# DiltheyLab/HLA-LA

Measured on AMD Instinct MI355X. Metric: paired reads/sec aligned to PRG graph, higher is better.
Workload: dtype int32

## Files before the change

hla-la_amd/csrc/kernel_dp.hip:

```cpp
#include "batch.h"
#include "../../include/hlala_gpu.h"

namespace hlala {

enum { K_DIAG = 0, K_GGAP = 1, K_SGAP = 2, K_HOP = 3, K_JUMP = 4 };
enum { M_D = 0, M_GG = 1, M_SG = 2 };
enum { PH_IDLE = 0, PH_RUN, PH_SELECT, PH_BT, PH_EXPAND, PH_DONE };

constexpr u64 HKEY_EMPTY = ~0ull;
#ifndef HLALA_DP_PROFILE_LOG2
#define HLALA_DP_PROFILE_LOG2 18
#endif
#ifndef HLALA_EARLY_GEN_MAX
#define HLALA_EARLY_GEN_MAX 0xFFFFFE
#endif
constexpr int DP_EARLY_GEN_MAX = HLALA_EARLY_GEN_MAX;
constexpr int EXT_PENDING = 0x7FFFFFFF;
constexpr int DP_BT_STEPS_PER_TRIP = 32;

#ifndef HLALA_DP_TAIL_THREADS
#define HLALA_DP_TAIL_THREADS 128
#endif
constexpr int DP_TAIL_THREADS = HLALA_DP_TAIL_THREADS;
#ifndef HLALA_DP_TINY_WAVES
#define HLALA_DP_TINY_WAVES 4
#endif
#ifndef HLALA_DP_WIDE_THREADS
#define HLALA_DP_WIDE_THREADS 64
#endif
#ifndef HLALA_DP_BROAD_THREADS
#define HLALA_DP_BROAD_THREADS HLALA_DP_TAIL_THREADS
#endif
#ifndef HLALA_DP_LARGE_THREADS
#define HLALA_DP_LARGE_THREADS HLALA_DP_TAIL_THREADS
#endif
#ifndef HLALA_DP_HUGE_THREADS
#define HLALA_DP_HUGE_THREADS HLALA_DP_TAIL_THREADS
#endif
struct DpTiny  { static constexpr bool JF = false; static constexpr int THREADS = 64, WAVES = HLALA_DP_TINY_WAVES, GW = 16, WCAP = 16,   HC = 32,   IBITS = 4,  CELLS = 2048,     EARLY = 4096,     IMPCAP = 64,   COMPLETED = 256,          STEPS = 1024;     typedef u32 Best; typedef short Slot; typedef unsigned char ImpIdx; static constexpr bool IN_MEMORY = false; };
#ifndef HLALA_DP_TINYJF_WAVES
#define HLALA_DP_TINYJF_WAVES 4
#endif
struct DpTinyJF : DpTiny { static constexpr bool JF = true; static constexpr int WAVES = HLALA_DP_TINYJF_WAVES; };
struct DpMid   { static constexpr bool JF = false; static constexpr int THREADS = 64, WAVES = 4, GW = 32, WCAP = 32,   HC = 128,  IBITS = 5,  CELLS = 4096,     EARLY = 8192,     IMPCAP = 256,  COMPLETED = 512,          STEPS = 2048;     typedef u32 Best; typedef short Slot; typedef unsigned short ImpIdx; static constexpr bool IN_MEMORY = false; };
struct DpSmall { static constexpr bool JF = false; static constexpr int THREADS = 64, WAVES = 5, GW = 64, WCAP = 64,   HC = 128,  IBITS = 7,  CELLS = DP_CELLS, EARLY = DP_CELLS, IMPCAP = 2048, COMPLETED = DP_COMPLETED, STEPS = DP_STEPS; typedef u32 Best; typedef short Slot; typedef unsigned short ImpIdx; static constexpr bool IN_MEMORY = false; };
struct DpWide  { static constexpr bool JF = false; static constexpr int THREADS = HLALA_DP_WIDE_THREADS, WAVES = 2, GW = HLALA_DP_WIDE_THREADS, WCAP = 256,  HC = 512,  IBITS = 8,  CELLS = DP_CELLS, EARLY = DP_CELLS, IMPCAP = 2048, COMPLETED = DP_COMPLETED, STEPS = DP_STEPS; typedef u32 Best; typedef short Slot; typedef unsigned short ImpIdx; static constexpr bool IN_MEMORY = false; };
struct DpBroad { static constexpr bool JF = false; static constexpr int THREADS = HLALA_DP_BROAD_THREADS, WAVES = 1, GW = HLALA_DP_BROAD_THREADS, WCAP = 512,  HC = 1024, IBITS = 9,  CELLS = DP_CELLS_LARGE, EARLY = DP_CELLS_LARGE, IMPCAP = 4096, COMPLETED = DP_COMPLETED_LARGE, STEPS = DP_STEPS; typedef u32 Best; typedef int Slot; typedef unsigned short ImpIdx; static constexpr bool IN_MEMORY = false; };
struct DpLarge { static constexpr bool JF = false; static constexpr int THREADS = HLALA_DP_LARGE_THREADS, WAVES = 1, GW = HLALA_DP_LARGE_THREADS, WCAP = 1024, HC = 2048, IBITS = 10, CELLS = DP_CELLS_LARGE, EARLY = DP_CELLS_LARGE, IMPCAP = 4096, COMPLETED = DP_COMPLETED_LARGE, STEPS = DP_STEPS; typedef u32 Best; typedef int Slot; typedef unsigned short ImpIdx; static constexpr bool IN_MEMORY = false; };

struct DpHuge  { static constexpr bool JF = false; static constexpr int THREADS = HLALA_DP_HUGE_THREADS, WAVES = 1, GW = HLALA_DP_HUGE_THREADS, WCAP = 8192, HC = 16384, IBITS = 13, CELLS = 131072, EARLY = 131072, IMPCAP = 8192, COMPLETED = 65536, STEPS = DP_STEPS; typedef u64 Best; typedef int Slot; typedef unsigned short ImpIdx; static constexpr bool IN_MEMORY = true; };
#ifndef HLALA_DP_SORT_SCRATCH
#define HLALA_DP_SORT_SCRATCH 4096
#endif
constexpr int DP_SORT_SCRATCH = HLALA_DP_SORT_SCRATCH;

struct DpState {
    int itemIdx;
    int item, rOff, seqLen, start_seq, startLevel, startNode;
    int d, b1, b2, n1, n2, nCells, nCompleted, curMax, firstMaxSlot, lastInc, earlyInit, itersRun, diagonals;
    int earlyMaxNat;
    u32 cellsEvaluated;
    int endSlot, endScore, nSteps, nCols;
    int have, sb, se, err;
    int isAlias;
    int needTier;
};

template <bool SMALL> struct TlistT { typedef unsigned short type; };
template <> struct TlistT<true> { typedef unsigned char type; };

template <class C>
struct __align__(16) DpLdsT {
    u64 hkey[C::HC];
    typename C::Best hbest[3][C::HC];
    typename TlistT<(C::HC <= 256)>::type tlist[C::HC];
    u64 fkey[2][C::WCAP];
    typename C::Slot fslot[2][C::WCAP];
    short fD[2][C::WCAP], fG[2][C::WCAP], fS[2][C::WCAP];
    typename C::Slot tes[C::HC];
    unsigned char timp[C::HC];
    typename C::ImpIdx hq[C::HC];
    int nNew, nImp, nKeepF, err, nCompletedAdd;
    int chunkNext, chunkEnd;
    int jumpMet;
    int nTa;
    int nextPhase;
    int btSlot, btM, btX, btY, btGuard, btDone;
    DpState st;
    u64 accCalls, accIters, accCells, accEdges;
#ifdef HLALA_DP_TIMING
    long long tPh[16];
#endif
#ifdef HLALA_DP_PROFILE
    long long pfStart; int pfSlow, pfImp, pfPre, pfMaxNT, pfMaxF; long long pfPh[16];
#endif
};

struct __align__(16) CellRec { u64 key; short sc[4]; u32 bt[3]; u32 pad; };

template <class C>
struct DpSlabT {
    char* base;
    static constexpr size_t O_CELL      = 0;
    static constexpr size_t O_EARLY_KEY = O_CELL + (size_t)C::CELLS * 32;
    static constexpr size_t O_STEP_XY   = O_EARLY_KEY + (size_t)C::EARLY * 8;
    static constexpr size_t O_IMP_KEY   = O_STEP_XY + (size_t)C::STEPS * 8;
    static constexpr size_t O_IMP_NEW   = O_IMP_KEY + (size_t)C::IMPCAP * 8;
// ... 127 lines not shown
template <int GW> __device__ __forceinline__ u64 grp_ballot(bool p)
{
    static_assert(GW <= 64, "grp_ballot: one wavefront at most (grp_any / grp_rank for blocks)");
    u64 b = __ballot(p);
    if(GW == 64) return b;
    return (b >> grp_base<GW>()) & ((1ull << (GW & 63)) - 1ull);
}
template <int GW> __device__ __forceinline__ bool grp_any(bool p)
{
    if constexpr (GW > 64) {
        const int w = __ballot(p) != 0 ? 1 : 0; int* x = blk_words<GW>();
        if(lane_id() == 0) x[threadIdx.x >> 6] = w;
        blk_barrier();
        int r = 0;
#pragma unroll
        for(int i = 0; i < BlkX<GW>::NW; i++) r |= x[i];
        blk_barrier();
        return r != 0;
    } else return grp_ballot<GW>(p) != 0;
}
template <int GW> __device__ __forceinline__ int grp_rank(bool p, int& total)
{
    if constexpr (GW > 64) {
        const u64 m = __ballot(p);
        const int off = (int)__builtin_amdgcn_mbcnt_hi((u32)(m >> 32), __builtin_amdgcn_mbcnt_lo((u32)m, 0u));
        int* x = blk_words<GW>(); const int wv = (int)(threadIdx.x >> 6);
        if(lane_id() == 0) x[wv] = __popcll(m);
        blk_barrier();
        int before = 0, tot = 0;
#pragma unroll
        for(int i = 0; i < BlkX<GW>::NW; i++) { const int t = x[i]; if(i < wv) before += t; tot += t; }
        blk_barrier();
        total = tot;
        return before + off;
    } else {
        const u64 m = grp_ballot<GW>(p);
        total = __popcll(m);
        return __popcll(m & ((1ull << grp_lane<GW>()) - 1ull));
    }
}
template <int GW> __device__ __forceinline__ int grp_bcast0(int v)
{
    if(GW == 64) return __builtin_amdgcn_readfirstlane(v);
    if constexpr (GW > 64) {
        int* x = blk_words<GW>();
        if(threadIdx.x == 0) x[0] = v;
        blk_barrier();
        const int r = x[0];
        blk_barrier();
        return __builtin_amdgcn_readfirstlane(r);
    } else return __shfl(v, grp_base<GW>());
}
template <int GW> __device__ __forceinline__ int guni(int v) { return GW >= 64 ? __builtin_amdgcn_readfirstlane(v) : v; }

template <class C> __device__ __forceinline__ void dp_sync()
{
#if defined(__AMDGCN_TGSPLIT__) || defined(__gfx950_tgsplit__)
#error "kernel_dp.hip: dp_sync releases at workgroup scope -- build with -DHLALA_DP_AGENT_RELEASE for threadgroup-split mode"
#endif
#ifdef HLALA_DP_AGENT_RELEASE
#define DP_RELEASE_SCOPE "agent"
#else
#define DP_RELEASE_SCOPE "workgroup"
#endif
    if constexpr (C::IN_MEMORY) { __builtin_amdgcn_fence(__ATOMIC_RELEASE, DP_RELEASE_SCOPE); if constexpr (C::GW > 64) __builtin_amdgcn_s_barrier(); else __builtin_amdgcn_wave_barrier(); __builtin_amdgcn_fence(__ATOMIC_ACQUIRE, "agent"); }
    else if constexpr (C::GW > 64) blk_barrier();
    else { WSYNC(); }
}
#define DSYNC() dp_sync<C>()

__device__ __forceinline__ u64 mk_key(int x, int y, int node) { return ((u64)(u32)x << 40) | ((u64)(u32)y << 28) | (u64)(u32)node; }
__device__ __forceinline__ int key_x(u64 k) { return (int)(k >> 40); }
__device__ __forceinline__ int key_y(u64 k) { return (int)((k >> 28) & 0xFFF); }
__device__ __forceinline__ int key_node(u64 k) { return (int)(k & 0xFFFFFFF); }
__device__ __forceinline__ u32 hash64(u64 k)
{
    const u32 node = (u32)k & 0xFFFFFFFu, y = (u32)(k >> 28) & 0xFFFu, x = (u32)(k >> 40);
    u32 h = node + __umul24(y, 17u) + __umul24(x, 31u);
    return h ^ (h >> 6) ^ (h >> 12);
}

__device__ __forceinline__ u32 hash_mix(u64 k)
{
    u32 h = (u32)k * 0x9E3779B1u ^ (u32)(k >> 32) * 0x85EBCA77u;
    h ^= h >> 15; h *= 0x2C1B3C6Du; h ^= h >> 12;
    return h;
}

template <class C> __device__ __forceinline__ u32 tgt_hash(u64 k) { return (C::HC > 256 ? hash_mix(k) : hash64(k)) & (u32)(C::HC - 1); }

template <class C>
__device__ inline int dp_find(const DpLdsT<C>& S, u64 key)
{
    u32 h = tgt_hash<C>(key);
#pragma nounroll
    for(int probe = 0; probe < C::HC; probe++) {
        const u64 cur = S.hkey[h];
        if(cur == key) return (int)h;
        if(cur == HKEY_EMPTY) return -1;
        h = (h + 1) & (C::HC - 1);
    }
    return -1;
}

__device__ __forceinline__ u32 mk_bt(int prev, int src, int kind, int edge) { return (u32)prev | ((u32)src << 17) | ((u32)kind << 19) | (((u32)edge & 0xFFu) << 22); }
__device__ __forceinline__ int bt_prev(u32 b) { return (int)(b & 0x1FFFF); }
// ... 158 lines not shown
    const int gl = grp_lane<GW>();
    for(int i = gl; i < C::HC; i += GW) { S.hkey[i] = HKEY_EMPTY; S.hbest[0][i] = 0; S.hbest[1][i] = 0; S.hbest[2][i] = 0; }
    if(gl == 0) {
        DpState& st = S.st;
        st.itemIdx = itemIdx;
        st.item = it.item; st.rOff = it.rOff; st.seqLen = it.seqLen; st.start_seq = it.start_seq; st.startLevel = it.startLevel; st.startNode = it.startNode;
        st.diagonals = it.seqLen + G.L - 1;
        st.d = 1; st.b1 = 0; st.b2 = 1; st.n1 = 1; st.n2 = 0; st.nCells = 1; st.nCompleted = 0;
        st.curMax = 0; st.firstMaxSlot = 0; st.lastInc = 0; st.earlyInit = 0; st.earlyMaxNat = -1; st.itersRun = 0;
        st.cellsEvaluated = 0;
        st.endSlot = -1; st.endScore = 0; st.nSteps = 0; st.nCols = 0;
        st.have = 0; st.sb = 0; st.se = -1; st.err = 0; st.needTier = 0; st.isAlias = 0;
        S.err = 0; S.nTa = 0; S.jumpMet = 0;
#ifdef HLALA_DP_PROFILE
        S.pfStart = clock64(); S.pfSlow = 0; S.pfImp = 0; S.pfPre = 0; S.pfMaxNT = 0; S.pfMaxF = 0; for(int i = 0; i < 16; i++) S.pfPh[i] = 0;
#endif
        CellRec c0; c0.key = mk_key(it.startLevel, it.start_seq, it.startNode);
        c0.sc[0] = 0; c0.sc[1] = (short)DP_NEG; c0.sc[2] = (short)DP_NEG; c0.sc[3] = 0; c0.bt[0] = 0; c0.bt[1] = 0; c0.bt[2] = 0; c0.pad = 0;
        sl.cell()[0] = c0;
        S.fkey[0][0] = mk_key(it.startLevel, it.start_seq, it.startNode); S.fslot[0][0] = 0;
        S.fD[0][0] = 0; S.fG[0][0] = (short)DP_NEG; S.fS[0][0] = (short)DP_NEG;
    }
    DSYNC();
    return PH_RUN;
}

template <class C>
__device__ inline int dp_iterate(DpLdsT<C>& S, const DpSlabT<C>& sl, const DevGraph& G, const int4* nrec, const uint8_t* readBases, const bool fwd, int& edgesAcc, u64* sortScratch)
{
    constexpr int GW = C::GW;
    const int gl = grp_lane<GW>();
    DpState& st = S.st;
    const int dir = fwd ? 1 : -1;
    const int seqLen = guni<GW>(st.seqLen);
    const int max_levelI = G.L - 1, max_seqI = seqLen;
    const int limitY = fwd ? seqLen : 0;
    const int d = guni<GW>(st.d);
    const int n1 = guni<GW>(st.n1), n2 = guni<GW>(st.n2);
    const int b1 = guni<GW>(st.b1), b2 = guni<GW>(st.b2), bn = b2;
    const int lastInc0 = guni<GW>(st.lastInc), diagonals = guni<GW>(st.diagonals);
    const uint8_t* seqp = readBases + guni<GW>(st.rOff);

    if(d > diagonals || (d - lastInc0) > 40) return PH_SELECT;
    if(n1 == 0 && n2 == 0) {
        int last = lastInc0 + 40; if(last > diagonals) last = diagonals;
        if(gl == 0) st.itersRun = last;
        DSYNC();
        return PH_SELECT;
    }
    if(d > 60000) { if(gl == 0) { st.itersRun = d; st.err = __LINE__; } DSYNC(); return PH_DONE; }

#if defined(HLALA_DP_TIMING)
    long long tq0 = clock64();
#define DP_TQ(i) do { __builtin_amdgcn_s_waitcnt(0); long long t_ = clock64(); if(gl == 0) S.tPh[i] += t_ - tq0; tq0 = t_; } while(0)
#elif defined(HLALA_DP_PROFILE)
    long long tq0 = clock64();
#define DP_TQ(i) do { __builtin_amdgcn_s_waitcnt(0); long long t_ = clock64(); if(gl == 0) S.pfPh[i] += t_ - tq0; tq0 = t_; } while(0)
#else
#define DP_TQ(i) do { } while(0)
#endif
    const int* eoff = fwd ? G.out_off : G.in_off; const int* eto = fwd ? G.out_to : G.in_from; const uint8_t* elab = fwd ? G.out_label : G.in_label;
    const int* joff = fwd ? G.jf_off : G.jb_off; const int* jnode = fwd ? G.jf_node : G.jb_node; const int* jlvl = fwd ? G.jf_lvl : G.jb_lvl;
    const uint8_t* eprk = fwd ? G.out_prank : G.in_prank; const uint8_t* jprk = fwd ? G.jf_prank : G.jb_prank;
    int edges = 0;
    const int nMax = n1 > n2 ? n1 : n2;
    constexpr bool APPEND = (GW >= 64) && (C::WCAP > 64);
    typedef typename TlistT<(C::HC <= 256)>::type TlT;
    int nTa = 0;
    auto append = [&](const bool claimed, const u32 h) {
        if constexpr (APPEND && GW == 64) {
            const u64 m = __ballot(claimed);
            if(claimed) S.tlist[nTa + (int)__builtin_amdgcn_mbcnt_hi((u32)(m >> 32), __builtin_amdgcn_mbcnt_lo((u32)m, 0u))] = (TlT)h;
            nTa += __popcll(m);
        } else if constexpr (APPEND) {
            const u64 m = __ballot(claimed);
            if(m) {
                int base = 0;
                if(lane_id() == 0) base = atomicAdd(&S.nTa, (int)__popcll(m));
                base = __builtin_amdgcn_readfirstlane(base);
                const int pos = base + (int)__builtin_amdgcn_mbcnt_hi((u32)(m >> 32), __builtin_amdgcn_mbcnt_lo((u32)m, 0u));
                if(claimed && pos < C::HC) S.tlist[pos] = (TlT)h;
            }
        }
    };
    for(int i = gl; i < nMax; i += GW) {
        const bool hasA = i < n2, hasB = i < n1;
        u64 pkA = hasA ? S.fkey[b2][i] : 0, pkB = hasB ? S.fkey[b1][i] : 0;
        const int pxA = key_x(pkA), pyA = key_y(pkA), nodeA = key_node(pkA);
        const int pxB = key_x(pkB), pyB = key_y(pkB), nodeB = key_node(pkB);
        const int nxA = pxA + dir, nyA = pyA + dir;
        const bool doA = hasA && !(nxA > max_levelI || nyA > max_seqI || nxA < 0 || nyA < 0);
        const int pDA = hasA ? (int)S.fD[b2][i] : 0;
        const int pD = hasB ? (int)S.fD[b1][i] : 0, pG = hasB ? (int)S.fG[b1][i] : 0, pS = hasB ? (int)S.fS[b1][i] : 0;
        int4 ra0 = make_int4(0, 0, 0, 0), ra1 = ra0, rb0 = ra0, rb1 = ra0; unsigned char rc = 0;
        if(doA) { ra0 = nrec[2 * (size_t)nodeA]; ra1 = nrec[2 * (size_t)nodeA + 1]; rc = fwd ? seqp[pyA] : seqp[pyA - 1]; }
        if(hasB) { rb0 = nrec[2 * (size_t)nodeB]; rb1 = nrec[2 * (size_t)nodeB + 1]; }
        const int a0 = ra0.x, degA = ra0.y & 0xFFFF, tnA0 = ra0.z, tnA1 = ra0.w;
        const unsigned char labA0 = (unsigned char)(ra1.w & 0xFF), labA1 = (unsigned char)((ra1.w >> 8) & 0xFF);
        const int rkA1 = (ra1.w >> 16) & 1, rkB1 = (rb1.w >> 16) & 1;
        const int e0 = rb0.x, degB = rb0.y & 0xFFFF, tnB0 = rb0.z, tnB1 = rb0.w;
        const int j0 = rb1.x, j1 = j0 + (int)((u32)rb0.y >> 16), jn0 = rb1.y, jx0 = rb1.z;
        const unsigned char labB0 = (unsigned char)(rb1.w & 0xFF), labB1 = (unsigned char)((rb1.w >> 8) & 0xFF);
        DP_TQ(4);
        const int ord0 = (1 << (C::IBITS + 8)) | (i << 8);
        const int nyG = pyB + dir, nxB = pxB + dir;
        const bool okA = doA, okB = hasB;
// ... 316 lines not shown
            if(keep && Dv == curMax0 && diff != 0) anyEqDiff = true;
            if(keep) { if(Dv > itMaxNew) { itMaxNew = Dv; itMaxKey = key; } else if(Dv == itMaxNew && key < itMaxKey) itMaxKey = key; }
            if(act) {
                S.hbest[0][h] = keep ? (typename C::Best)(u32)slot : (typename C::Best)0xFFFFFFFFu;
                S.hbest[1][h] = (typename C::Best)(((u32)(unsigned short)(short)mD) | ((u32)(unsigned short)(short)mG << 16));
                S.hbest[2][h] = (typename C::Best)(u32)(unsigned short)(short)mS;
            }
            DP_TQ(13);
        }
        DSYNC();
    }
    anyEqDiff = grp_any<GW>(anyEqDiff); anyOw = grp_any<GW>(anyOw);
    {
        const int mine = itMaxNew;
        itMaxNew = grp_max_i32<GW>(mine);
        if(itMaxNew > curMax0) itMaxKey = grp_min_u64<GW>(mine == itMaxNew ? itMaxKey : ~0ull);
    }
    DP_TQ(6);
    if(guni<GW>(S.err)) { if(gl == 0) { st.itersRun = d; st.err = __LINE__; } DSYNC(); return PH_DONE; }
    const int nCompletedNew = nCompleted0 + guni<GW>(S.nCompletedAdd);
    if constexpr (!C::JF) {
        int nImp = guni<GW>(S.nImp);
        for(int q = gl; q < nImp; q += GW) {
            int es = sl.imp_slot()[q]; int msk = sl.imp_mask()[q];
            for(int m = 0; m < 3; m++) if(msk & (1 << m)) { sl.cell()[es].sc[m] = sl.imp_new()[4 * q + m]; sl.cell()[es].bt[m] = sl.imp_bt()[3 * q + m]; }
        }
        if(nImp) {
            DSYNC();
            for(int i = gl; i < n1; i += GW) {
                const int ph = dp_find<C>(S, S.fkey[b1][i]);
                if(ph >= 0) { const int q = (int)S.hq[ph]; if(q < C::IMPCAP && q < nImp) { S.fD[b1][i] = sl.imp_new()[4 * q + 0]; S.fG[b1][i] = sl.imp_new()[4 * q + 1]; S.fS[b1][i] = sl.imp_new()[4 * q + 2]; } }
            }
        }
    }
    int curMax = curMax0, lastInc = lastInc0, firstMaxSlot = -1;
    if(itMaxNew > curMax0) {
        curMax = itMaxNew; lastInc = d;
        int fs = -1;
        for(int t = gl; t < nT; t += GW) { int h = S.tlist[t]; if(S.hkey[h] == itMaxKey) fs = (int)S.hbest[0][h]; }
        firstMaxSlot = grp_max_i32<GW>(fs);
    }
    if(anyEqDiff || anyOw) lastInc = d;
    int earlyMaxNat = earlyMaxNat0;
    if constexpr (!C::JF) if(earlyInit) { const int m = grp_max_i32<GW>(earlyNatMax); if(m > earlyMaxNat) earlyMaxNat = m; }

    DP_TQ(1);
    int mx = itMaxNew;
    if constexpr (!C::JF) if(slow) {
        mx = DP_NEG;
        for(int t = gl; t < nT; t += GW) { int h = S.tlist[t]; if((u32)S.hbest[0][h] != 0xFFFFFFFFu) { int v = (short)((u32)S.hbest[1][h] & 0xFFFF); mx = max(mx, v); } }
        mx = grp_max_i32<GW>(mx);
    }
    int nNew = 0;
    for(int t0 = 0; t0 < nT; t0 += GW) {
        int t = t0 + gl;
        bool pass = false; u64 key = 0; int h = 0;
        if(t < nT) { h = S.tlist[t]; key = S.hkey[h]; if((u32)S.hbest[0][h] != 0xFFFFFFFFu) { int v = (short)((u32)S.hbest[1][h] & 0xFFFF); pass = (mx - v) <= 15; } }
        int passTot; const int pos = nNew + grp_rank<GW>(pass, passTot);
        if(pass && pos < C::WCAP) {
            S.fkey[bn][pos] = key; S.fslot[bn][pos] = (typename C::Slot)(int)S.hbest[0][h];
            S.fD[bn][pos] = (short)((u32)S.hbest[1][h] & 0xFFFF); S.fG[bn][pos] = (short)((u32)S.hbest[1][h] >> 16); S.fS[bn][pos] = (short)((u32)S.hbest[2][h] & 0xFFFF);
        }
        nNew += passTot;
    }
    if(nNew > C::WCAP) { if(gl == 0) { st.itersRun = d; st.err = __LINE__; st.needTier = tier_for_frontier(nNew); } DSYNC(); return PH_DONE; }
    DSYNC();
    const bool wideSort = C::WCAP > GW && nNew > GW;
    if(wideSort) for(int t = gl; t < nT; t += GW) { int h = S.tlist[t]; S.hkey[h] = HKEY_EMPTY; S.hbest[0][h] = 0; S.hbest[1][h] = 0; S.hbest[2][h] = 0; }
    if(nNew > 1 && nNew <= GW) {
        const bool act = gl < nNew;
        u64 key = 0; typename C::Slot vs = 0; short vD = 0, vG = 0, vS = 0; int rank = 0;
        if(act) {
            key = S.fkey[bn][gl]; vs = S.fslot[bn][gl]; vD = S.fD[bn][gl]; vG = S.fG[bn][gl]; vS = S.fS[bn][gl];
            for(int u = 0; u < nNew; u++) rank += (S.fkey[bn][u] < key) ? 1 : 0;
        }
        DSYNC();
        if(act) { S.fkey[bn][rank] = key; S.fslot[bn][rank] = vs; S.fD[bn][rank] = vD; S.fG[bn][rank] = vG; S.fS[bn][rank] = vS; }
    } else if(wideSort) {
        DSYNC();
        int Pn = GW * 2; while(Pn < nNew) Pn <<= 1;
        u64* keys; u64* pay;
        if constexpr (C::IN_MEMORY) {
            if(Pn <= DP_SORT_SCRATCH) { keys = sortScratch; pay = sortScratch + DP_SORT_SCRATCH; }
            else { keys = sl.sort_spill(); pay = keys + C::WCAP; }
        } else { keys = &S.fkey[bn][0]; pay = (u64*)&S.hbest[2][0]; }
        auto enc = [](int v) -> u64 { return v == DP_NEG ? 0ull : (u64)(u32)(v + 64); };
        auto dec = [](u64 e) -> short { return e == 0 ? (short)DP_NEG : (short)((int)e - 64); };
        for(int i = gl; i < Pn; i += GW) {
            if(i < nNew) {
                pay[i] = ((u64)(u32)(int)S.fslot[bn][i] << 36) | (enc(S.fD[bn][i]) << 24) | (enc(S.fG[bn][i]) << 12) | enc(S.fS[bn][i]);
                if constexpr (C::IN_MEMORY) keys[i] = S.fkey[bn][i];
            } else { keys[i] = ~0ull; pay[i] = 0; }
        }
        DSYNC();
        for(int k = 2; k <= Pn; k <<= 1)
            for(int j = k >> 1; j > 0; j >>= 1) {
                for(int idx = gl; idx < (Pn >> 1); idx += GW) {
                    const int i = ((idx & ~(j - 1)) << 1) | (idx & (j - 1)), l = i | j;
                    const bool up = (i & k) == 0;
                    const u64 ka = keys[i], kb = keys[l];
                    if((ka > kb) == up) { const u64 pa = pay[i], pb = pay[l]; keys[i] = kb; keys[l] = ka; pay[i] = pb; pay[l] = pa; }
                }
                if constexpr (C::IN_MEMORY) { if(Pn <= DP_SORT_SCRATCH) { if constexpr (GW > 64) blk_barrier(); else { WSYNC(); } } else DSYNC(); }
                else DSYNC();
            }
        for(int i = gl; i < Pn; i += GW) {
            const u64 pv = pay[i];
            if(i < nNew) {
                S.fD[bn][i] = dec((pv >> 24) & 0xFFF); S.fG[bn][i] = dec((pv >> 12) & 0xFFF); S.fS[bn][i] = dec(pv & 0xFFF); S.fslot[bn][i] = (typename C::Slot)(int)(pv >> 36);
                if constexpr (C::IN_MEMORY) S.fkey[bn][i] = keys[i];
            }
            if constexpr (!C::IN_MEMORY) pay[i] = 0;
        }
    }
    DSYNC();
    if(!wideSort) for(int t = gl; t < nT; t += GW) { int h = S.tlist[t]; S.hkey[h] = HKEY_EMPTY; S.hbest[0][h] = 0; S.hbest[1][h] = 0; S.hbest[2][h] = 0; }
    if(gl == 0) {
        st.b2 = b1; st.b1 = bn;
        st.n2 = n1; st.n1 = nNew;
        st.d = d + 1; st.itersRun = d;
        st.nCells = nCells; st.nCompleted = nCompletedNew; st.earlyInit = earlyInit; st.earlyMaxNat = earlyMaxNat;
        st.curMax = curMax; st.lastInc = lastInc; if(firstMaxSlot >= 0) st.firstMaxSlot = firstMaxSlot;
        st.cellsEvaluated += (u32)nT;
#ifdef HLALA_DP_PROFILE
        if(slow) S.pfSlow++; S.pfImp += S.nImp; if(prepass) S.pfPre++; if(nT > S.pfMaxNT) S.pfMaxNT = nT; if(nNew > S.pfMaxF) S.pfMaxF = nNew;
#endif
    }
    DSYNC();
    DP_TQ(2);
    return PH_RUN;
}

template <class C>
__device__ inline int dp_select_many(const DpSlabT<C>& sl, const DevGraph& G, int nCompleted, int best, int selectedIndex)
{
    constexpr int GW = C::GW;
    const int gl = grp_lane<GW>();
    int found = -1;
    int nt = 0;
    for(int i0 = 0; i0 < nCompleted; i0 += GW) {
        int i = i0 + gl; bool tie = false; int s = 0; u64 kk = 0;
        if(i < nCompleted) { s = sl.completed()[i]; if(sl.cell()[s].sc[0] == best) { tie = true; u64 k = sl.cell()[s].key; kk = xz_key(key_x(k), key_node(k) - G.level_off[key_x(k)]); } }
        int tieTot; const int rk = grp_rank<GW>(tie, tieTot);
        if(tie) { const int pos = nt + rk; sl.tie_slot()[pos] = s; sl.tie_key()[pos] = kk; }
        nt += tieTot;
    }
    dp_sync<C>();
    u64 prefix = 0; int k = selectedIndex;
    for(int bit = 51; bit >= 0; bit--) {
        int cnt = 0;
        for(int i = gl; i < nt; i += GW) { const u64 kk = sl.tie_key()[i]; if((kk >> (bit + 1)) == (prefix >> (bit + 1)) && !((kk >> bit) & 1ull)) cnt++; }
        cnt = grp_sum_i32<GW>(cnt);
        if(k >= cnt) { k -= cnt; prefix |= 1ull << bit; }
    }
    for(int i = gl; i < nt; i += GW) if(sl.tie_key()[i] == prefix) found = sl.tie_slot()[i];
    return found;
}

template <class C>
__device__ inline int dp_select(DpLdsT<C>& S, const DpSlabT<C>& sl, const DevGraph& G, u32 rng_seed, const bool fwd)
{
    constexpr int GW = C::GW;
    const int gl = grp_lane<GW>();
    DpState& st = S.st;
    const int nCompleted = guni<GW>(st.nCompleted);
    const u32 seed = rng_seed + (u32)guni<GW>(st.item);
    const int curMax = guni<GW>(st.curMax), firstMaxSlot = guni<GW>(st.firstMaxSlot), start_seq = guni<GW>(st.start_seq);
    int endSlot = -1, endScore = 0;
    if(GW <= 64 && nCompleted > 0 && nCompleted <= GW) {
// ... 324 lines not shown
    const DpItem* items[DP_POOL_MAX];
    const uint8_t* bases[DP_POOL_MAX];
};

template <class C, int TIER>
__device__ __forceinline__ void dp_class_run(const DevGraph& G, const DevBatch& B, const DpItem* __restrict__ items, DpLdsT<C>& S, DpSlabT<C> sl, u64* sortScratch, const u32 rng_seed,
                                             const int4* __restrict__ nrecOut, const int4* __restrict__ nrecIn, const uint8_t* __restrict__ readBases);

template <class C, int TIER>
__global__ __launch_bounds__(C::THREADS, C::WAVES) void k_dp(const DevGraph* __restrict__ Gp, const DevBatch* __restrict__ Bp, const DpItem* __restrict__ items,
                                                        char* slabs, size_t slabBytes, u32 rng_seed,
                                                        const int4* __restrict__ nrecOut, const int4* __restrict__ nrecIn, const uint8_t* __restrict__ readBasesArg, const DpPoolArgs pool)
{
    constexpr int GW = C::GW;
    constexpr int NG = GW >= 64 ? 1 : 64 / GW;
    static_assert(C::THREADS == (GW >= 64 ? GW : 64), "block size");
    const DevGraph& G = *Gp;
    const int g = (int)((threadIdx.x & 63) / GW);
    DpLdsT<C>* Sp; DpSlabT<C> sl; u64* sortScratch = nullptr;
    if constexpr (C::IN_MEMORY) {
        __shared__ u64 scratch[2 * DP_SORT_SCRATCH];
        char* base = slabs + (size_t)blockIdx.x * slabBytes;
        Sp = (DpLdsT<C>*)base; sl.base = base + ((sizeof(DpLdsT<C>) + 255) & ~(size_t)255); sortScratch = scratch;
    } else {
        __shared__ DpLdsT<C> SS[NG];
        Sp = &SS[g]; sl.base = slabs + ((size_t)blockIdx.x * NG + g) * slabBytes;
    }
    if constexpr (TIER >= DP_POOL_TIER) {
        const int nB = __builtin_amdgcn_readfirstlane(pool.n);
        for(int bi = 0; bi < nB; bi++) {
            dp_class_run<C, TIER>(G, *pool.B[bi], pool.items[bi], *Sp, sl, sortScratch, pool.seed[bi], nrecOut, nrecIn, pool.bases[bi]);
            DSYNC();
        }
    } else dp_class_run<C, TIER>(G, *Bp, items, *Sp, sl, sortScratch, rng_seed, nrecOut, nrecIn, readBasesArg);
}

template <class C, int TIER>
__device__ __forceinline__ void dp_class_run(const DevGraph& G, const DevBatch& B, const DpItem* __restrict__ items, DpLdsT<C>& S, DpSlabT<C> sl, u64* sortScratch, const u32 rng_seed,
                                             const int4* __restrict__ nrecOut, const int4* __restrict__ nrecIn, const uint8_t* __restrict__ readBases)
{
    constexpr int GW = C::GW;
    constexpr int NG = GW >= 64 ? 1 : 64 / GW;
#ifndef HLALA_DP_DRAW0
#define HLALA_DP_DRAW0 8
#endif
    constexpr int DRAW = (TIER == 0 && C::JF) ? HLALA_DP_DRAW0 : 1;
    const int gl = grp_lane<GW>();

    if(gl == 0) { S.accCalls = 0; S.accIters = 0; S.accCells = 0; S.accEdges = 0; }
#ifdef HLALA_DP_TIMING
    if(gl == 0) { for(int i = 0; i < 16; i++) S.tPh[i] = 0; }
#endif
#ifdef HLALA_DP_TIMING
    long long tAcc[6] = {0, 0, 0, 0, 0, 0}; long long trips = 0, runGroups = 0; long long tMark = clock64();
#define DP_T(i) do { long long t_ = clock64(); tAcc[i] += t_ - tMark; tMark = t_; } while(0)
#else
#define DP_T(i) do { } while(0)
#endif

    constexpr int NPASS = (TIER == 0 && !C::JF) ? 4 : 2;
    for(int pass = 0; pass < NPASS; pass++) {
        const int dirPass = pass & 1;
        const bool foPass = pass >= 2;
        int* fetchCounter = foPass ? &B.work_counter[WC_FO_FETCH + dirPass]
                          : &B.work_counter[TIER == 0 ? (C::JF ? 4 + dirPass : (dirPass ? 10 : 1)) : 13 + 4 * (TIER - 1) + 2 * dirPass];
        const int seg = (C::JF ? DPL_JF : DPL_GEN) + dirPass;
        const bool dense = TIER == 0 && !foPass;
        const int segStart = dense ? uni(B.dp_blk[(size_t)seg * B.dp_nblk]) : 0;
        const int nItems = dense ? uni(B.dp_blk[(size_t)(seg + 1) * B.dp_nblk]) - segStart
                         : (foPass ? uni(B.work_counter[WC_FO_COUNT + dirPass]) : uni(B.work_counter[12 + 4 * (TIER > 0 ? TIER - 1 : 0) + 2 * dirPass]));
        const int* srcList = dense ? B.dp_list + segStart
                           : (foPass ? B.retry_list + (size_t)(14 + dirPass) * (size_t)B.n_chains
                           : B.retry_list + (size_t)(2 * (TIER > 0 ? TIER - 1 : 0) + dirPass) * (size_t)B.n_chains);
        const bool fwd = dirPass != 0;
        if constexpr (DRAW > 1) { if(gl == 0) { S.chunkNext = 0; S.chunkEnd = 0; } DSYNC(); }
        int phase = PH_IDLE;
        bool more = true;
        int edgesAcc = 0;

        for(;;) {
            if(phase == PH_RUN) phase = dp_iterate<C>(S, sl, G, fwd ? nrecOut : nrecIn, readBases, fwd, edgesAcc, sortScratch);
            DP_T(5);
            if(phase == PH_SELECT) phase = dp_select<C>(S, sl, G, rng_seed, fwd);
            DP_T(4);
            if(phase == PH_BT) phase = dp_backtrace<C>(S, sl, DP_BT_STEPS_PER_TRIP, fwd);
            DP_T(3);
            if(phase == PH_EXPAND) phase = dp_expand<C>(S, sl, G, B, fwd ? nrecOut : nrecIn, fwd);
            DP_T(2);
            if(phase == PH_DONE) {
                const int edges = grp_sum_i32<GW>(edgesAcc);
                if(gl == 0) {
                    DpState& st = S.st;
                    S.nextPhase = PH_IDLE;
#ifdef HLALA_DP_PROFILE
                    if(B.dbg && TIER == HLALA_DP_PROFILE && !C::JF) {
                        const long long cyc = clock64() - S.pfStart;
                        if(cyc > (1ll << HLALA_DP_PROFILE_LOG2) && (HLALA_DP_PROFILE_LOG2 >= 12 || (((u32)st.item * 2654435761u) >> 24) == 0)) { int q = atomicAdd(&B.dbg[0], 1); if(q < 500) { int* r = B.dbg + 16 + 16 * q; r[0] = st.item; r[1] = st.itersRun; r[2] = (int)st.cellsEvaluated; r[3] = st.nCells;
                            r[4] = S.pfSlow; r[5] = S.pfImp; r[6] = S.pfPre; r[7] = (int)(cyc >> 10); r[8] = S.pfMaxNT;
                            r[9] = (int)(S.pfPh[4] >> 10); r[10] = (int)(S.pfPh[5] >> 10); r[11] = (int)(S.pfPh[0] >> 10); r[12] = (int)(S.pfPh[3] >> 10); r[13] = (int)(S.pfPh[6] >> 10); r[14] = (int)(S.pfPh[1] >> 10); r[15] = (int)(S.pfPh[2] >> 10); } }
                    }
#endif
                    const bool capacity = st.err != 0 && st.err > -1000000;
                    bool handed = false;
                    if constexpr (C::JF && TIER == 0) if(capacity && S.jumpMet) {
                        if(st.isAlias) ((int*)(items + st.itemIdx))[0] = st.item;
                        const int q = atomicAdd(&B.work_counter[WC_FO_COUNT + dirPass], 1); B.retry_list[(size_t)(14 + dirPass) * (size_t)B.n_chains + q] = st.itemIdx;
                        atomicAdd(&B.work_counter[WC_JF_FAILED], 1);
                        handed = true;
                    }
                    if(handed) { }
                    else if(capacity && TIER < DP_LAST_TIER) {
                        int to = TIER + 1; if(st.needTier > to) to = st.needTier; if(to > DP_LAST_TIER) to = DP_LAST_TIER;
                        int* cnt = &B.work_counter[12 + 4 * (to - 1) + 2 * dirPass]; int* lst = B.retry_list + (size_t)(2 * (to - 1) + dirPass) * (size_t)B.n_chains;
                        if(st.isAlias) ((int*)(items + st.itemIdx))[0] = st.item;
                        int q = atomicAdd(cnt, 1); lst[q] = st.itemIdx;
                        if(to >= DP_SIDE_TIER && B.n_pairs > 0 && !B.unpaired) B.pair_deferred[B.chain_read[st.item >> 1] >> 1] = 1;
                    } else {
                        const int item = st.item;
                        B.dp_iters[item] = st.itersRun; B.dp_score[item] = st.have ? st.endScore : INT32_MIN;
                        B.dp_ncols[item] = st.have ? st.nCols : -1; B.dp_sb[item] = st.sb; B.dp_se[item] = st.se; B.dp_err[item] = st.err;
                        S.accCalls++; S.accIters += (u64)st.itersRun; S.accCells += (u64)st.cellsEvaluated; S.accEdges += (u64)edges;
                        int nx = B.dp_alias_head[item]; if(nx < 0) nx = B.dp_alias_next[item];
                        const bool failed = st.err != 0 && st.err > -1000000;
                        while(nx >= 0 && failed) {
                            B.dp_iters[nx] = st.itersRun; B.dp_score[nx] = INT32_MIN; B.dp_ncols[nx] = -1; B.dp_sb[nx] = st.sb; B.dp_se[nx] = st.se; B.dp_err[nx] = st.err;
                            S.accCalls++; S.accIters += (u64)st.itersRun; S.accCells += (u64)st.cellsEvaluated; S.accEdges += (u64)edges;
                            nx = B.dp_alias_next[nx];
                        }
                        if(nx >= 0) {
                            st.item = nx; st.isAlias = 1;
                            st.endSlot = -1; st.endScore = 0; st.nSteps = 0; st.nCols = 0; st.have = 0; st.sb = 0; st.se = -1; st.err = 0;
                            S.nextPhase = PH_SELECT;
                        }
                    }
                }
                DSYNC();
                phase = guni<GW>(S.nextPhase);
            }
            DP_T(1);
            if(phase == PH_IDLE && more) {
                int w = 0;
                if(gl == 0) {
                    if constexpr (DRAW > 1) {
                        int nx = S.chunkNext;
                        if(nx >= S.chunkEnd) { nx = atomicAdd(fetchCounter, DRAW); S.chunkEnd = nx + DRAW; }
                        S.chunkNext = nx + 1; w = nx;
                    } else w = atomicAdd(fetchCounter, 1);
                }
                w = grp_bcast0<GW>(w);
                if(w >= nItems) more = false;
                else {
                    const int idx = guni<GW>(srcList[w]);
                    const int4* ip = (const int4*)(items + idx);
                    int4 a = ip[0], b = ip[1];
                    DpItem it; it.item = a.x; it.rOff = a.y; it.seqLen = a.z; it.start_seq = a.w; it.startLevel = b.x; it.startNode = b.y; it.pad0 = 0; it.pad1 = 0;
                    phase = dp_begin<C>(S, sl, G, it, idx);
                    edgesAcc = 0;
                }
            }
            DP_T(0);
            if(!__ballot(phase != PH_IDLE)) break;
#ifdef HLALA_DP_TIMING
            trips++; runGroups += __popcll(__ballot(phase == PH_RUN)) / GW;
#endif
            DP_T(5);
        }
    }
    if(gl == 0 && S.accCalls) {
        atomicAdd(&B.counters[CNT_DP_CALLS], S.accCalls); atomicAdd(&B.counters[CNT_DP_ITERS], S.accIters);
        atomicAdd(&B.counters[CNT_DP_CELLS], S.accCells); atomicAdd(&B.counters[CNT_EDGES], S.accEdges);
    }
#ifdef HLALA_DP_TIMING
    if(TIER == 0 && (threadIdx.x & 63) == 0) { for(int i = 0; i < 8; i++) atomicAdd(&B.counters[24 + i], (u64)S.tPh[i]); for(int i = 0; i < 8; i++) atomicAdd(&B.counters[16 + i], (u64)S.tPh[8 + i]);
        for(int i = 0; i < 6; i++) atomicAdd(&B.counters[8 + i], (u64)tAcc[i]); atomicAdd(&B.counters[14], (u64)trips); atomicAdd(&B.counters[15], (u64)runGroups); }
#endif
}

template <int PER>
__device__ __forceinline__ void stitch_rounds(const DevBatch& B, const DevTables& T, const size_t cb, const int rOff, const int total, const int padL, const int nL, const int nSeed,
                                              const int nR, const int newEnd, const int stride, const int lane, double& llOut, int& f0, int& f1, int& l0, int& l1)
{
    const int seedAt = padL + nL, rightAt = seedAt + nSeed, padRAt = rightAt + nR;
    const int srcShift = (stride - nR) - rightAt;
    double carry = 0.0; int baseIdx = 0;
    f0 = -1; f1 = -1; l0 = -1; l1 = -1;
    for(int c0 = 0; c0 < total; c0 += 64 * PER) {
        const int chunk = min(64 * PER, total - c0);
        const int per = (chunk + 63) / 64;
        const int j0 = c0 + lane * per, j1 = min(c0 + chunk, j0 + per);
        int lv[PER], ed[PER]; unsigned char gcv[PER], scv[PER], kind[PER];
#pragma unroll
        for(int k = 0; k < PER; k++) {
            const int j = j0 + k; const bool in = k < per && j < j1;
            lv[k] = -1; ed[k] = -1; gcv[k] = '_'; scv[k] = '_'; kind[k] = 4;
            if(in) {
                if(j < padL) { kind[k] = 0; scv[k] = B.read_bases[rOff + j]; }
                else if(j < seedAt) { kind[k] = 1; lv[k] = B.ext_level[cb + j]; gcv[k] = B.ext_g[cb + j]; scv[k] = B.ext_s[cb + j]; }
                else if(j < rightAt) { const int q = j - seedAt; kind[k] = 2; lv[k] = B.seed_level[cb + q]; ed[k] = B.seed_edge[cb + q]; gcv[k] = B.seed_g[cb + q]; scv[k] = B.seed_s[cb + q]; }
                else if(j < padRAt) { const size_t p = cb + j + srcShift; kind[k] = 3; lv[k] = B.ext_level[p]; ed[k] = B.ext_edge[p]; gcv[k] = B.ext_g[p]; scv[k] = B.ext_s[p]; }
                else { kind[k] = 0; scv[k] = B.read_bases[rOff + newEnd + 1 + (j - padRAt)]; }
            }
        }
        WSYNC();
        int nb = 0;
#pragma unroll
        for(int k = 0; k < PER; k++) if(kind[k] != 4 && scv[k] != '_') nb++;
        int tot; const int before = baseIdx + wave_excl_scan(nb, tot);
        unsigned char qv[PER];
        {
            int idx = before;
#pragma unroll
            for(int k = 0; k < PER; k++) {
                qv[k] = 0;
                if(kind[k] != 4 && scv[k] != '_') { if(gcv[k] != '_') qv[k] = B.read_quals[rOff + idx]; idx++; }
            }
        }
#pragma unroll
        for(int k = 0; k < PER; k++) {
            const size_t o = cb + j0 + k;
            if(kind[k] == 1) B.ext_fromseed[o] = 0;
            else if(kind[k] != 4) {
                if(kind[k] != 3 || srcShift != 0) { B.ext_level[o] = lv[k]; B.ext_edge[o] = ed[k]; B.ext_g[o] = gcv[k]; B.ext_s[o] = scv[k]; }
                B.ext_fromseed[o] = kind[k] == 2 ? 1 : 0;
            }
        }
        double t1[PER], t2[PER];
// ... 135 lines not shown
```

Before: 5.549 million.

## Sort DP frontier in registers with packed bitonic network for wide tiers

```diff
diff --git a/hla-la_amd/csrc/kernel_dp.hip b/hla-la_amd/csrc/kernel_dp.hip
--- a/hla-la_amd/csrc/kernel_dp.hip
+++ b/hla-la_amd/csrc/kernel_dp.hip
@@ -53,6 +53,9 @@
 #define HLALA_DP_SORT_SCRATCH 4096
 #endif
 constexpr int DP_SORT_SCRATCH = HLALA_DP_SORT_SCRATCH;
+#ifndef HLALA_DP_REG_SORT_SPAN
+#define HLALA_DP_REG_SORT_SPAN 0x7FFFFFFF
+#endif
 
 struct DpState {
     int itemIdx;
@@ -286,6 +289,75 @@
     } else return __shfl(v, grp_base<GW>());
 }
 template <int GW> __device__ __forceinline__ int guni(int v) { return GW >= 64 ? __builtin_amdgcn_readfirstlane(v) : v; }
+template <int GW> __device__ __forceinline__ void grp_max2_i32(int& a, int& b)
+{
+    static_assert(GW >= 64, "grp_max2_i32: groups of whole wavefronts");
+    a = wave_max_i32(a); b = wave_max_i32(b);
+    if constexpr (GW > 64) {
+        int* x = blk_words<GW>(); const int wv = (int)(threadIdx.x >> 6);
+        if(lane_id() == 0) { x[2 * wv] = a; x[2 * wv + 1] = b; }
+        blk_barrier();
+        a = x[0]; b = x[1];
+#pragma unroll
+        for(int i = 1; i < BlkX<GW>::NW; i++) { a = op_max_(a, x[2 * i]); b = op_max_(b, x[2 * i + 1]); }
+        blk_barrier();
+    }
+}
+
+template <int M> __device__ __forceinline__ u32 lane_xor_u32(u32 v)
+{
+    if constexpr (M == 1) return (u32)__builtin_amdgcn_update_dpp((int)v, (int)v, 0xB1, 0xF, 0xF, false);
+    else if constexpr (M == 2) return (u32)__builtin_amdgcn_update_dpp((int)v, (int)v, 0x4E, 0xF, 0xF, false);
+    else if constexpr (M < 32) return (u32)__builtin_amdgcn_ds_swizzle((int)v, 0x1F | (M << 10));
+    else { static_assert(M == 32, "lane_xor_u32: within one wavefront"); const auto r = __builtin_amdgcn_permlane32_swap(v, v, false, false); return lane_id() < 32 ? r[1] : r[0]; }
+}
+template <int M> __device__ __forceinline__ u64 lane_xor_u64(u64 v) { return ((u64)lane_xor_u32<M>((u32)(v >> 32)) << 32) | (u64)lane_xor_u32<M>((u32)v); }
+
+template <int N> struct IntC { static constexpr int value = N; };
+template <int GW, int E, int K, int J>
+__device__ __forceinline__ void reg_bitonic_stage(u64 (&v)[E], const int gl, u64* xs)
+{
+    if constexpr (J < E) {
+#pragma unroll
+        for(int r = 0; r < E; r++) {
+            if(r & J) continue;
+            bool up;
+            if constexpr (K < E) up = (r & K) == 0; else if constexpr (K == GW * E) up = true; else up = (gl & (K / E)) == 0;
+            const u64 a = v[r], b = v[r | J];
+            if((a > b) == up) { v[r] = b; v[r | J] = a; }
+        }
+    } else {
+        constexpr int M = J / E;
+        const bool up = (K == GW * E) ? true : (gl & (K / E)) == 0;
+        const bool keepMin = up == ((gl & M) == 0);
+        u64 p[E];
+        if constexpr (M < 64) {
+#pragma unroll
+            for(int r = 0; r < E; r++) p[r] = lane_xor_u64<M>(v[r]);
+        } else {
+            static_assert(GW == 128 && M == 64, "reg_bitonic_stage: groups of at most two wavefronts");
+#pragma unroll
+            for(int r = 0; r < E; r++) xs[r * GW + gl] = v[r];
+            blk_barrier();
+#pragma unroll
+            for(int r = 0; r < E; r++) p[r] = xs[r * GW + (gl ^ 64)];
+        }
+#pragma unroll
+        for(int r = 0; r < E; r++) if((p[r] < v[r]) == keepMin) v[r] = p[r];
+    }
+}
+template <int GW, int E, int K, int J>
+__device__ __forceinline__ void reg_bitonic_merge(u64 (&v)[E], const int gl, u64* xs)
+{
+    reg_bitonic_stage<GW, E, K, J>(v, gl, xs);
+    if constexpr (J > 1) reg_bitonic_merge<GW, E, K, J / 2>(v, gl, xs);
+}
+template <int GW, int E, int K = 2>
+__device__ __forceinline__ void reg_bitonic_sort(u64 (&v)[E], const int gl, u64* xs)
+{
+    reg_bitonic_merge<GW, E, K, K / 2>(v, gl, xs);
+    if constexpr (K < GW * E) reg_bitonic_sort<GW, E, K * 2>(v, gl, xs);
+}
 
 template <class C> __device__ __forceinline__ void dp_sync()
 {
@@ -550,6 +622,7 @@
 
 #if defined(HLALA_DP_TIMING)
     long long tq0 = clock64();
+    if(gl == 0) S.tPh[15]++;
 #define DP_TQ(i) do { __builtin_amdgcn_s_waitcnt(0); long long t_ = clock64(); if(gl == 0) S.tPh[i] += t_ - tq0; tq0 = t_; } while(0)
 #elif defined(HLALA_DP_PROFILE)
     long long tq0 = clock64();
@@ -972,21 +1045,91 @@
         mx = grp_max_i32<GW>(mx);
     }
     int nNew = 0;
+    constexpr bool REG = !C::IN_MEMORY && C::WCAP > GW;
+    constexpr int IB = C::IBITS + 1;
+    static_assert(!REG || ((1 << IB) == C::HC && GW >= 64), "REG classes: HC = 2 WCAP, groups of whole wavefronts");
+    typedef typename C::Slot SlotT;
+    int xlo = 0x7FFFFFFF, xhi = -1;
     for(int t0 = 0; t0 < nT; t0 += GW) {
         int t = t0 + gl;
         bool pass = false; u64 key = 0; int h = 0;
         if(t < nT) { h = S.tlist[t]; key = S.hkey[h]; if((u32)S.hbest[0][h] != 0xFFFFFFFFu) { int v = (short)((u32)S.hbest[1][h] & 0xFFFF); pass = (mx - v) <= 15; } }
         int passTot; const int pos = nNew + grp_rank<GW>(pass, passTot);
-        if(pass && pos < C::WCAP) {
-            S.fkey[bn][pos] = key; S.fslot[bn][pos] = (typename C::Slot)(int)S.hbest[0][h];
+        if constexpr (REG) {
+            if(pass && pos < C::WCAP) { S.fkey[bn][pos] = key; S.fslot[bn][pos] = (SlotT)h; xlo = min(xlo, key_x(key)); xhi = max(xhi, key_x(key)); }
+            else if(t < nT) { S.hkey[h] = HKEY_EMPTY; S.hbest[0][h] = 0; S.hbest[1][h] = 0; S.hbest[2][h] = 0; }
+        } else if(pass && pos < C::WCAP) {
+            S.fkey[bn][pos] = key; S.fslot[bn][pos] = (SlotT)(int)S.hbest[0][h];
             S.fD[bn][pos] = (short)((u32)S.hbest[1][h] & 0xFFFF); S.fG[bn][pos] = (short)((u32)S.hbest[1][h] >> 16); S.fS[bn][pos] = (short)((u32)S.hbest[2][h] & 0xFFFF);
         }
         nNew += passTot;
     }
     if(nNew > C::WCAP) { if(gl == 0) { st.itersRun = d; st.err = __LINE__; st.needTier = tier_for_frontier(nNew); } DSYNC(); return PH_DONE; }
+    constexpr int XB = 24 - IB;
+    bool regFit = false;
+    if constexpr (REG) if(nNew > GW) { int a = xhi, b = -xlo; grp_max2_i32<GW>(a, b); xhi = a; xlo = -b; regFit = xhi - xlo <= (1 << XB) - 2 && xhi - xlo <= HLALA_DP_REG_SORT_SPAN; }
     DSYNC();
+    DP_TQ(7);
+    if constexpr (REG) {
+        auto emit = [&](const int pos, const u64 key, const int h) {
+            const u32 s0 = (u32)S.hbest[0][h], s1 = (u32)S.hbest[1][h], s2 = (u32)S.hbest[2][h];
+            S.fkey[bn][pos] = key; S.fslot[bn][pos] = (SlotT)(int)s0;
+            S.fD[bn][pos] = (short)(s1 & 0xFFFF); S.fG[bn][pos] = (short)(s1 >> 16); S.fS[bn][pos] = (short)(s2 & 0xFFFF);
+            S.hkey[h] = HKEY_EMPTY; S.hbest[0][h] = 0; S.hbest[1][h] = 0; S.hbest[2][h] = 0;
+        };
+        if(nNew <= GW) {
+            const bool act = gl < nNew;
+            u64 key = 0; int h = 0, rank = 0;
+            if(act) {
+                key = S.fkey[bn][gl]; h = (int)S.fslot[bn][gl];
+                for(int u = 0; u < nNew; u++) rank += (S.fkey[bn][u] < key) ? 1 : 0;
+            }
+            DSYNC();
+            DP_TQ(14);
+            if(act) emit(rank, key, h);
+        } else if(regFit) {
+            int Pn = GW * 2; while(Pn < nNew) Pn <<= 1;
+            auto regSort = [&](auto eTag) {
+                constexpr int E = decltype(eTag)::value, XS = 40 + IB;
+                u64 v[E];
+#pragma unroll
+                for(int r = 0; r < E; r++) {
+                    const int i = gl * E + r;
+                    v[r] = ~0ull;
+                    if(i < nNew) { const u64 key = S.fkey[bn][i]; v[r] = ((u64)(u32)(key_x(key) - xlo) << XS) | ((key & 0xFFFFFFFFFFull) << IB) | (u64)(u32)(int)S.fslot[bn][i]; }
+                }
+                static_assert(GW == 64 || sizeof(S.tes) >= sizeof(u64) * C::WCAP, "the cross-wave stage exchanges through tes[]");
+                reg_bitonic_sort<GW, E>(v, gl, (u64*)&S.tes[0]);
+                DP_TQ(14);
+#pragma unroll
+                for(int r = 0; r < E; r++) {
+                    const int i = gl * E + r;
+                    if(i < nNew) emit(i, ((u64)(u32)(xlo + (int)(v[r] >> XS)) << 40) | ((v[r] >> IB) & 0xFFFFFFFFFFull), (int)(v[r] & (u64)(C::HC - 1)));
+                }
+            };
+            if(Pn == 2 * GW) regSort(IntC<2>());
+            else if(Pn == 4 * GW) regSort(IntC<4>());
+            else if constexpr (C::WCAP >= 8 * GW) regSort(IntC<8>());
+        } else {
+            int Pn = GW * 2; while(Pn < nNew) Pn <<= 1;
+            for(int i = nNew + gl; i < Pn; i += GW) { S.fkey[bn][i] = ~0ull; S.fslot[bn][i] = 0; }
+            DSYNC();
+            for(int k = 2; k <= Pn; k <<= 1)
+                for(int j = k >> 1; j > 0; j >>= 1) {
+                    for(int idx = gl; idx < (Pn >> 1); idx += GW) {
+                        const int i = ((idx & ~(j - 1)) << 1) | (idx & (j - 1)), l = i | j;
+                        const u64 ka = S.fkey[bn][i], kb = S.fkey[bn][l];
+                        if((ka > kb) == ((i & k) == 0)) { const SlotT pa = S.fslot[bn][i], pb = S.fslot[bn][l]; S.fkey[bn][i] = kb; S.fkey[bn][l] = ka; S.fslot[bn][i] = pb; S.fslot[bn][l] = pa; }
+                    }
+                    DSYNC();
+                }
+            DP_TQ(14);
+            for(int i = gl; i < nNew; i += GW) emit(i, S.fkey[bn][i], (int)S.fslot[bn][i]);
+        }
+    } else {
     const bool wideSort = C::WCAP > GW && nNew > GW;
     if(wideSort) for(int t = gl; t < nT; t += GW) { int h = S.tlist[t]; S.hkey[h] = HKEY_EMPTY; S.hbest[0][h] = 0; S.hbest[1][h] = 0; S.hbest[2][h] = 0; }
+    DP_TQ(2);
     if(nNew > 1 && nNew <= GW) {
         const bool act = gl < nNew;
         u64 key = 0; typename C::Slot vs = 0; short vD = 0, vG = 0, vS = 0; int rank = 0;
@@ -1034,7 +1177,9 @@
         }
     }
     DSYNC();
+    DP_TQ(14);
     if(!wideSort) for(int t = gl; t < nT; t += GW) { int h = S.tlist[t]; S.hkey[h] = HKEY_EMPTY; S.hbest[0][h] = 0; S.hbest[1][h] = 0; S.hbest[2][h] = 0; }
+    }
     if(gl == 0) {
         st.b2 = b1; st.b1 = bn;
         st.n2 = n1; st.n1 = nNew;
@@ -1465,6 +1610,9 @@
     if(gl == 0) { for(int i = 0; i < 16; i++) S.tPh[i] = 0; }
 #endif
 #ifdef HLALA_DP_TIMING
+#ifndef HLALA_DP_TIMING_TIER
+#define HLALA_DP_TIMING_TIER 0
+#endif
     long long tAcc[6] = {0, 0, 0, 0, 0, 0}; long long trips = 0, runGroups = 0; long long tMark = clock64();
 #define DP_T(i) do { long long t_ = clock64(); tAcc[i] += t_ - tMark; tMark = t_; } while(0)
 #else
@@ -1510,7 +1658,7 @@
                         const long long cyc = clock64() - S.pfStart;
                         if(cyc > (1ll << HLALA_DP_PROFILE_LOG2) && (HLALA_DP_PROFILE_LOG2 >= 12 || (((u32)st.item * 2654435761u) >> 24) == 0)) { int q = atomicAdd(&B.dbg[0], 1); if(q < 500) { int* r = B.dbg + 16 + 16 * q; r[0] = st.item; r[1] = st.itersRun; r[2] = (int)st.cellsEvaluated; r[3] = st.nCells;
                             r[4] = S.pfSlow; r[5] = S.pfImp; r[6] = S.pfPre; r[7] = (int)(cyc >> 10); r[8] = S.pfMaxNT;
-                            r[9] = (int)(S.pfPh[4] >> 10); r[10] = (int)(S.pfPh[5] >> 10); r[11] = (int)(S.pfPh[0] >> 10); r[12] = (int)(S.pfPh[3] >> 10); r[13] = (int)(S.pfPh[6] >> 10); r[14] = (int)(S.pfPh[1] >> 10); r[15] = (int)(S.pfPh[2] >> 10); } }
+                            r[9] = (int)(S.pfPh[4] >> 10); r[10] = (int)(S.pfPh[5] >> 10); r[11] = (int)(S.pfPh[0] >> 10); r[12] = (int)(S.pfPh[3] >> 10); r[13] = (int)(S.pfPh[6] >> 10); r[14] = (int)(S.pfPh[1] >> 10); r[15] = (int)((S.pfPh[2] + S.pfPh[7] + S.pfPh[14]) >> 10); } }
                     }
 #endif
                     const bool capacity = st.err != 0 && st.err > -1000000;
@@ -1584,7 +1732,7 @@
         atomicAdd(&B.counters[CNT_DP_CELLS], S.accCells); atomicAdd(&B.counters[CNT_EDGES], S.accEdges);
     }
 #ifdef HLALA_DP_TIMING
-    if(TIER == 0 && (threadIdx.x & 63) == 0) { for(int i = 0; i < 8; i++) atomicAdd(&B.counters[24 + i], (u64)S.tPh[i]); for(int i = 0; i < 8; i++) atomicAdd(&B.counters[16 + i], (u64)S.tPh[8 + i]);
+    if(TIER == HLALA_DP_TIMING_TIER && (threadIdx.x & 63) == 0) { for(int i = 0; i < 8; i++) atomicAdd(&B.counters[24 + i], (u64)S.tPh[i]); for(int i = 0; i < 8; i++) atomicAdd(&B.counters[16 + i], (u64)S.tPh[8 + i]);
         for(int i = 0; i < 6; i++) atomicAdd(&B.counters[8 + i], (u64)tAcc[i]); atomicAdd(&B.counters[14], (u64)trips); atomicAdd(&B.counters[15], (u64)runGroups); }
 #endif
 }
```

After: 5.608 million, median of 6. +1.1%, better.
